# apple/ml-gmpi

Hardware: NVIDIA H100
Metric: MPI frames/s (96 planes, 1024^2) (higher is better)
Workload: dtype f32

## Files before the change

__graft_entry__.py:

```python
import os
import sys

ROOT = os.path.dirname(os.path.abspath(__file__))
for p in (ROOT, os.path.join(ROOT, "oracle")):
    if p not in sys.path:
        sys.path.insert(0, p)


def build() -> None:
    import ml_gmpi_b200
    from ml_gmpi_b200 import _build, _lib
    path = _build.build_library(force=False)
    assert os.path.exists(path)
    lib = _lib.load()
    assert lib.gmpi_abi_version() == _lib.ABI_VERSION
    import mpi_oracle
    mpi_oracle.build()
    print(f"built {path} and {mpi_oracle._SO}")


def smoke() -> None:
    import numpy as np
    import torch
    import ml_gmpi_b200 as g
    from ml_gmpi_b200 import synth
    import mpi_oracle

    assert torch.cuda.is_available(), "smoke() needs a CUDA device"
    dev = torch.device("cuda:0")
    from ml_gmpi_b200 import _lib
    N, T, IMG = 16, 256, 256
    case = synth.make_case(n_planes=N, tex=T, img=IMG, n_mpi=2, views_per_mpi=2, seed=7, device="cpu", last_alpha_one=True)
    case = case.to(dev)
    assert _lib.load().gmpi_mpi_render_fwd_plan(4, N, T, T, IMG, IMG, None, None) == _lib.PLAN_STAGED
    rgba = case.rgba.clone().requires_grad_(True)
    mpi = g.MPI(align_corners=True, validate="full")
# ... 23 lines not shown
```

ml_gmpi_b200/__init__.py:

```python
from . import _lib
from ._build import build_library
from .mpi import (MPI, MPIOutOfPlaneError, Occupancy, build_occupancy, check_range, expand_factored, render_frames,
                  render_views, render_views_factored, unorm8_to_float)

__all__ = ["MPI", "MPIOutOfPlaneError", "render_views", "render_views_factored", "render_frames", "expand_factored", "check_range",
           "build_library", "build_occupancy", "Occupancy", "unorm8_to_float"]
```

ml_gmpi_b200/_build.py:

```python
import os
import shutil
import subprocess

PKG_DIR = os.path.dirname(os.path.abspath(__file__))
CSRC = os.path.join(PKG_DIR, "csrc")
LIB_PATH = os.path.join(PKG_DIR, "libgmpi_mpi_render.so")
SOURCES = ["mpi_render.cu", "mpi_skip.cu", "mpi_u8.cu"]
HEADERS = ["mpi_common.cuh", "mpi_fwd_staged.cuh", "mpi_fwd_direct.cuh", "mpi_kernel_keys.cuh", "mpi_bwd_box.cuh", "mpi_bwd_direct.cuh",
           "mpi_range_check.cuh", "mpi_light.cuh", "mpi_debug.cuh", "tma_utils.cuh", os.path.join("..", "..", "include", "gmpi_mpi_render.h")]
NVCC_FLAGS = ["-gencode", "arch=compute_90a,code=sm_90a", "-lineinfo", "-O3", "-std=c++17", "-diag-suppress", "1886", "-shared",
              "-Xcompiler", "-fPIC"]


def nvcc_path():
    p = shutil.which("nvcc") or "/usr/local/cuda/bin/nvcc"
    if not os.path.exists(p):
        raise RuntimeError("nvcc not found; cannot build the sm_90a library")
    return p


def is_stale(path: str = LIB_PATH) -> bool:
    if not os.path.exists(path):
        return True
    t = os.path.getmtime(path)
    deps = [os.path.join(CSRC, s) for s in SOURCES + HEADERS] + [os.path.join(CSRC, f) for f in os.listdir(CSRC)]
    return any(os.path.getmtime(d) > t for d in deps if os.path.isfile(d))


def _nvcc(args, verbose):
    res = subprocess.run([nvcc_path()] + args + (["-Xptxas", "-v"] if verbose else []), cwd=CSRC, capture_output=True, text=True)
    if res.returncode != 0:
        raise RuntimeError("nvcc failed:\n" + res.stdout + res.stderr)
    if verbose:
        print(res.stdout + res.stderr)


def build_library(force: bool = False, verbose: bool = False) -> str:
    if force or is_stale(LIB_PATH):
        _nvcc(NVCC_FLAGS + ["-o", LIB_PATH] + SOURCES, verbose)
    return LIB_PATH
```

ml_gmpi_b200/csrc/mpi_fwd_staged.cuh:

```cuda
#pragma once
#include "mpi_common.cuh"
#include "tma_utils.cuh"
#include "mpi_kernel_keys.cuh"

namespace gmpi {

constexpr int kConsWarps = 15;
constexpr int kPairs = 2;
constexpr int kPix = 2 * kPairs;
constexpr int kTileW = 64, kTileH = kPairs * kConsWarps;
constexpr int kConsThreads = kConsWarps * 32, kStagedThreads = kConsThreads + 32;
constexpr int kStages = 3, kStreamStages = 2;
constexpr int kRowsPerOp = 4;
constexpr int kMaxBW = 88;
constexpr int kMaxBH = (((kTileH * 5) / 4 + 6 + kRowsPerOp - 1) / kRowsPerOp) * kRowsPerOp;
constexpr int kMinBW = 56, kBWStep = 8;
constexpr int kNumMaps = (kMaxBW - kMinBW) / kBWStep + 1;
constexpr int kMaxPlanesStaged = 512;
constexpr int kWideBW = 96;

__host__ __device__ constexpr int class_width(int k, bool wide = false) { return wide && k == kNumMaps - 1 ? kWideBW : kMinBW + k * kBWStep; }

template <class E, class B, CUtensorMapDataType kType>
struct ElemBase {
// ... 11 lines not shown
    static __device__ __forceinline__ bool out_of_unit(uint32_t b) { return b > 0x3f800000u && b != 0x80000000u; }
};
template <> struct ElemTraits<__half> : ElemBase<__half, uint16_t, CU_TENSOR_MAP_DATA_TYPE_FLOAT16> {
    static __host__ __device__ constexpr int staged_width(int bw, bool factored) { return bw + (factored ? 32 : 8); }
    static __device__ __forceinline__ bool nonfinite(uint32_t b) { return (b & 0x7c00u) == 0x7c00u; }
    static __device__ __forceinline__ bool out_of_unit(uint32_t b) { return b > 0x3c00u && b != 0x8000u; }
};
template <> struct ElemTraits<uint8_t> : ElemBase<uint8_t, uint8_t, CU_TENSOR_MAP_DATA_TYPE_UINT8> {
    static __host__ __device__ constexpr int staged_width(int bw, bool) { return (bw + 12 + 15) & ~15; }
};

struct TmaMaps {
    CUtensorMap m[kNumMaps];
    CUtensorMap m8[kNumMaps], m16[kNumMaps], m32[kNumMaps];
    CUtensorMap rgb[kNumMaps], bg[kNumMaps], a[kNumMaps];
    CUtensorMap t;
};

struct __align__(16) StageMeta {
    int cx, cy;
    int rows2;
    int sel;
};

typedef float2 f2;
__device__ __forceinline__ f2 splat(float a) { return make_float2(a, a); }
__device__ __forceinline__ f2 mul2(f2 a, f2 b) { return make_float2(__fmul_rn(a.x, b.x), __fmul_rn(a.y, b.y)); }
__device__ __forceinline__ f2 add2(f2 a, f2 b) { return make_float2(__fadd_rn(a.x, b.x), __fadd_rn(a.y, b.y)); }
__device__ __forceinline__ f2 fma2(f2 a, f2 b, f2 c) { return make_float2(__fmaf_rn(a.x, b.x, c.x), __fmaf_rn(a.y, b.y, c.y)); }
__device__ __forceinline__ f2 add2_rm(f2 a, f2 b) { return make_float2(__fadd_rd(a.x, b.x), __fadd_rd(a.y, b.y)); }
constexpr float kFloorMagic = 12582912.0f;
constexpr int kFloorMagicBits = 0x4b400000;
constexpr int kSelSlow = 0;

__device__ __forceinline__ f2 div2_by_rcp(f2 a, f2 nb, f2 y) {
    const f2 q0 = mul2(a, y);
    const f2 r = fma2(q0, nb, a);
    return fma2(r, y, q0);
}

struct RayPairs {
    f2 rx2[kPairs], ry2[kPairs];
    f2 nrz[kPairs], yrz[kPairs];
};
__device__ __forceinline__ void pack_ray_pairs(const RayConst (&rc)[kPix], RayPairs& rp) {
#pragma unroll
// ... 177 lines not shown
    }
    __host__ __device__ __forceinline__ void split(int t, int per_view, int& v, int& pos) const {
        if (group == 1) { v = t / per_view; pos = t - v * per_view; return; }
        const int per_group = per_view * group, g = t / per_group, rem = t - g * per_group;
        pos = rem / group;
        v = g * group + (rem - pos * group);
    }
    __host__ __device__ __forceinline__ bool at(int j, TileXY& r) const {
        int pos;
        if (j < n1) {
            split(cta + j * grid, full_per_view, r.v, pos);
            r.px0 = (pos % tiles_x) * kTileW; r.py0 = (pos / tiles_x) * tile_h;
            return true;
        }
        if (p_step == 0) return false;
        const int u = p_start + (j - n1) * p_step;
        if (u >= n_part) return false;
        split(u, tiles_x, r.v, pos);
        r.px0 = pos * kTileW; r.py0 = full_rows * tile_h;
        return true;
    }
};

__device__ __forceinline__ void consumer_idle_tile(uint64_t* s_full, uint64_t* s_empty, int N, int n_stages, int lane, int& c_stage,
                                                   uint32_t& c_phase) {
    for (int i = 0; i < N; ++i) {
        const int s = c_stage;
        const uint32_t ph = c_phase;
        if (++c_stage == n_stages) { c_stage = 0; c_phase ^= 1u; }
        mbar_wait(&s_full[s], ph);
        __syncwarp();
        mbar_arrive_if(&s_empty[s], lane == 0);
    }
}

template <bool kFactored, class E>
struct FwdRing {
    static constexpr int kTileRows = kTileH, kRingStages = kStages, kBoxMaxH = kMaxBH;
    static constexpr int kPlaneFloats = ElemTraits<E>::staged_width(kFactored ? kWideBW : kMaxBW, kFactored) * kMaxBH * 4;
    static constexpr int kStride = kPlaneFloats;
    static constexpr size_t kStageBytes = (size_t)kPlaneFloats * sizeof(E);
    static constexpr bool kReverse = false;
    static constexpr bool kSleepPolls = false;
    static constexpr bool kWideFact = kFactored;
    static constexpr bool kBinaryCopies = true;
    static constexpr int kColourCopyRows = kMaxBH / 2;
    static_assert(kStages * kStageBytes + (size_t)kMaxPlanesStaged * 32 + 1024 <= 227 * 1024, "the ring must fit one SM");
};
static_assert(kMaxBH % 2 == 0 && kMaxBH / kRowsPerOp < 16, "half-height colour copies; binary digits of the chunk count");
static_assert(FwdRing<false, float>::kPlaneFloats == 15488 && FwdRing<true, float>::kPlaneFloats == 16896 &&
              FwdRing<false, __half>::kPlaneFloats == 16896 && FwdRing<true, __half>::kPlaneFloats == 22528 &&
              FwdRing<false, uint8_t>::kPlaneFloats == 19712, "the staged forward's ring stages");
static_assert(FwdRing<false, uint8_t>::kStageBytes % 128 == 0, "uint8 ring stages stay 128-byte aligned");

__host__ __device__ __forceinline__ int binary_copy_of_lane(int n_chunks, int lane, int& before) {
    const int bit = 3 - lane;
    before = (n_chunks >> (bit + 1)) << (bit + 1);
    return ((n_chunks >> bit) & 1) << bit;
}

constexpr int kStopSlots = 4;
constexpr uint32_t kAllConsumers = (1u << kConsWarps) - 1u;
static_assert(kStages <= kStopSlots, "stop-word slots must cover the producer's lead");
__device__ unsigned long long g_early_stop_skipped;

constexpr int kOccB = 8;
constexpr int kSelEmpty = 1 << 24;
struct OccMap {
    const uint32_t* bits;
    int words, rows;
    unsigned long long* skipped;
};
__host__ __device__ __forceinline__ int occ_words(int Wt) { return ((Wt + kOccB - 1) / kOccB + 31) / 32; }
__host__ __device__ __forceinline__ int occ_rows(int Ht) { return (Ht + kOccB - 1) / kOccB; }

constexpr int kOccThreads = 32 * kOccB;

__device__ __forceinline__ void store_occ_word(bool occupied, uint32_t* dst, uint32_t* s_w) {
    const int warp = threadIdx.x >> 5, lane = threadIdx.x & 31;
    const uint32_t b = __ballot_sync(0xffffffffu, occupied);
    const uint32_t nib = ((b & 0xffu) ? 1u : 0u) | ((b & 0xff00u) ? 2u : 0u) | ((b & 0xff0000u) ? 4u : 0u) | ((b & 0xff000000u) ? 8u : 0u);
    if (lane == 0) s_w[warp] = nib << (4 * warp);
    __syncthreads();
    if (threadIdx.x == 0) {
        uint32_t w = 0;
#pragma unroll
        for (int k = 0; k < kOccThreads / 32; ++k) w |= s_w[k];
// ... 19 lines not shown
#endif
        acc |= word & (0xffffffffu >> (31 - hi)) & (0xffffffffu << lo);
    }
    return acc;
}

__device__ __forceinline__ bool box_vote(int cx, int cy, int bw2, int rows2, const CoordPairs& c) {
    const f2 magic = splat(kFloorMagic);
    bool inbox = true;
#pragma unroll
    for (int P = 0; P < kPairs; ++P) {
        const f2 tx = add2_rm(c.ix[P], magic), ty = add2_rm(c.iy[P], magic);
        inbox = inbox && (unsigned)(__float_as_int(tx.x) - cx) <= (unsigned)bw2 && (unsigned)(__float_as_int(tx.y) - cx) <= (unsigned)bw2 &&
                (unsigned)(__float_as_int(ty.x) - cy) <= (unsigned)rows2 && (unsigned)(__float_as_int(ty.y) - cy) <= (unsigned)rows2;
    }
    return __all_sync(0xffffffffu, inbox);
}

__device__ __forceinline__ uint32_t idle_consumer_warps(int py0, int H) {
    const int live = (H - py0 + kPairs - 1) / kPairs;
    return live >= kConsWarps ? 0u : kAllConsumers & ~((1u << live) - 1u);
}

template <bool kAlignCorners, class Ring, bool kFact, bool kES = false, class E = float, bool kSkip = false>
__device__ __forceinline__ void staged_producer(const RenderParams& p, const TmaMaps& maps, E* s_buf, StageMeta* s_meta,
                                            uint64_t* s_full, uint64_t* s_empty, const TileWalk* s_walk, int lane,
                                            int n_stages = Ring::kRingStages, uint32_t* s_stop = nullptr, OccMap occ = OccMap{}) {
    constexpr bool kReverse = Ring::kReverse;
    constexpr int kStride = Ring::kStride;
    constexpr int kTileH = Ring::kTileRows, kMaxBH = Ring::kBoxMaxH, kStageFloats = Ring::kPlaneFloats;
    constexpr uint32_t kTBytes = kReverse ? (uint32_t)(kTileW * kTileH * 4) : 0u;
    const int Ht = p.Ht, Wt = p.Wt, N = p.N;
    const float fWt = (float)Wt, fHt = (float)Ht;
    const float hsx = 0.5f * (float)(Wt - 1), hsy = 0.5f * (float)(Ht - 1);
    const size_t img = (size_t)p.H * p.W;
    if (lane < kNumMaps) {
        if (kFact) { tma_prefetch_desc(&maps.rgb[lane]); tma_prefetch_desc(&maps.a[lane]); }
        else { tma_prefetch_desc(&maps.m[lane]); tma_prefetch_desc(&maps.m8[lane]); tma_prefetch_desc(&maps.m16[lane]); tma_prefetch_desc(&maps.m32[lane]); }
    }
    int p_stage = 0;
    uint32_t p_phase = 0;
    uint32_t n_skipped = 0;
    uint32_t n_empty = 0;
    TileXY txy;
    for (int j = 0; s_walk->at(j, txy); ++j) {
        const int v = txy.v, px0 = txy.px0, py0 = txy.py0;
        const int m = __ldg(p.view2mpi + v);
        uint32_t* const stop_word = kES ? s_stop + (j & (kStopSlots - 1)) : nullptr;
        float ev[3], zd[3];
        load_eye_z(p, v, ev, zd);
        const int cx = min(px0 + ((lane & 1) ? kTileW - 1 : 0), p.W - 1);
        const int cy = min(py0 + ((lane & 2) ? kTileH - 1 : 0), p.H - 1);
        float crx, cry, crz;
        load_ray(p, v, cx, cy, img, crx, cry, crz);
        const RayConst rc = make_ray_const(crx, cry, crz, ev, zd);
        for (int ii = 0; ii < N; ++ii) {
            const int i = kReverse ? N - 1 - ii : ii;
            const int s = p_stage;
            const uint32_t ph = p_phase;
            if (++p_stage == n_stages) { p_stage = 0; p_phase ^= 1u; }
            const PlaneConst pc = make_plane_const(p.dhw + ((size_t)m * N + i) * 3, ev[2]);
            const TexCoord tc = plane_coord<kAlignCorners>(pc, rc, hsx, hsy, fWt, fHt);
            const bool finite = fabsf(tc.ix) < 1e9f && fabsf(tc.iy) < 1e9f;
            const bool all_finite = __all_sync(0xffffffffu, finite);
            const int fx = finite ? (int)floorf(tc.ix) : 0, fy = finite ? (int)floorf(tc.iy) : 0;
            const int xmin = __reduce_min_sync(0xffffffffu, fx), xmax = __reduce_max_sync(0xffffffffu, fx);
            const int ymin = __reduce_min_sync(0xffffffffu, fy), ymax = __reduce_max_sync(0xffffffffu, fy);
            const int bx0 = ((xmin - 1) >> 2) << 2, by0 = ymin - 1;
            const int need_w = xmax - bx0 + 3, need_h = ymax - ymin + 4;
            int mode = 0;
            constexpr bool kWide = kFact && Ring::kWideFact;
            if (!all_finite || need_w > kMaxBW || ((need_h + kRowsPerOp - 1) / kRowsPerOp) * kRowsPerOp > kMaxBH) mode = 2;
            else if (bx0 > Wt - 1 || bx0 + need_w - 1 < 0 || by0 > Ht - 1 || by0 + need_h - 1 < 0) mode = 1;
            const int k = mode != 0 ? 0 : kWide ? (need_w <= 64 ? 1 : 4) : max(0, (need_w - kMinBW + kBWStep - 1) / kBWStep);
            const int bw = class_width(k, kWide);
            const int bxs = ElemTraits<E>::staged_origin(bx0), sw = ElemTraits<E>::staged_width(bw, kWide);
            const int n_ops = mode == 0 ? (need_h + kRowsPerOp - 1) / kRowsPerOp : 0;
            const int rows = n_ops * kRowsPerOp;
            const bool testable = kSkip && mode == 0 && pc.fast != 0.0f;
            uint32_t occ_bits = 0u;
            if (testable) occ_bits = occ_box_bits(occ.bits + ((size_t)m * N + i) * occ.rows * occ.words, Ht, Wt, occ.words, bx0, by0, bw, rows, lane);
            if (Ring::kSleepPolls) mbar_wait_sleep(&s_empty[s], ph ^ 1);
            else mbar_wait(&s_empty[s], ph ^ 1);
            bool empty = false;
            if constexpr (kSkip) {
                empty = testable && !__any_sync(0xffffffffu, occ_bits != 0u);
                n_empty += empty ? 1u : 0u;
            }
            bool skip = false;
            if constexpr (kES) {
                if (ii == 0) {
                    if (lane == 0) *stop_word = idle_consumer_warps(py0, p.H);
                } else {
                    skip = __shfl_sync(0xffffffffu, *(volatile uint32_t*)stop_word, 0) == kAllConsumers;
                    n_skipped += skip ? 1u : 0u;
                }
            }
            const int n_copy = skip || empty ? 0 : n_ops;
            if (lane == 0) {
                StageMeta mt;
                mt.cx = kFloorMagicBits + bx0; mt.cy = kFloorMagicBits + by0;
                mt.rows2 = rows - 2;
                mt.sel = bw | (mode << 8) | ((mode == 0 && pc.fast != 0.0f ? (1 << k) : kSelSlow) << 16) | ((bx0 - bxs) << 10);
                if (kSkip && empty) mt.sel |= kSelEmpty;
                if constexpr (kReverse) {
                    const int ext_x = min(px0 + kTileW - 1, p.W - 1) - px0, ext_y = min(py0 + kTileH - 1, p.H - 1) - py0;
                    if (Ring::kMagLimit * (xmax - xmin - 1) < ext_x || Ring::kMagLimit * (ymax - ymin - 1) < ext_y) mt.sel &= 0xffff;
                }
                s_meta[s] = mt;
                const uint32_t tx = (uint32_t)((kFact ? kMaxBH : rows) * sw * (int)(4 * sizeof(E)));
                if (n_copy > 0 || kTBytes) mbar_arrive_expect_tx(&s_full[s], (n_copy > 0 ? tx : 0u) + kTBytes);
                else mbar_arrive(&s_full[s]);
                if (kReverse)
// ... 45 lines not shown
}

__device__ __forceinline__ void store_tile_pixels(const RenderParams& p, int v, size_t img, int pxb, int py, int lane, float (&o)[4]) {
    if (p.options & kOptVec4Stores) {
        quad_transpose(o, lane);
        const int k = lane & 3, px = pxb + 4 * (lane >> 2);
        if (px >= p.W || py >= p.H) return;
        const float4 val = make_float4(o[0], o[1], o[2], o[3]);
        const size_t pix = (size_t)py * p.W + px;
        if (p.n_peers > 0) {
            const size_t fo = ((size_t)(p.frame_offset + v) * 4 + k) * img + pix;
            for (int r = 0; r < p.n_peers; ++r) *reinterpret_cast<float4*>(p.peer_frames[r] + fo) = val;
        } else {
            float* dst = k < 3 ? p.color + ((size_t)v * 3 + k) * img + pix : p.depth + (size_t)v * img + pix;
            *reinterpret_cast<float4*>(dst) = val;
        }
        return;
    }
    const int px = pxb + lane;
    if (px >= p.W || py >= p.H) return;
    store_pixel(p, v, img, (size_t)py * p.W + px, o[0], o[1], o[2], o[3]);
}

template <bool kAlignCorners, bool kEmitT, bool kFactored, bool kES, class E = float, bool kSkip = false>
__device__ __forceinline__ void fwd_staged_body(const RenderParams& p, const TmaMaps& maps, const int tiles_x, const int ring_stages,
                                                uint32_t* s_stop, OccMap occ = OccMap{}) {
    extern __shared__ __align__(1024) unsigned char smem_raw[];
    E* s_buf = reinterpret_cast<E*>(smem_raw);
    using Ring = FwdRing<kFactored, E>;
    static_assert(!(kFactored && std::is_same<E, uint8_t>::value), "uint8 MPIs are expanded");
    constexpr int kStages = Ring::kRingStages;
    const int n_stages = kFactored ? kStages : ring_stages;
    constexpr int kRingFloats = Ring::kPlaneFloats;
    constexpr int kAOff = kFactored ? 3 * (kRingFloats / 4) : 0;
    PlaneConst* s_pc = reinterpret_cast<PlaneConst*>(smem_raw + (size_t)n_stages * kRingFloats * sizeof(E));
    __shared__ StageMeta s_meta[kStages];
    __shared__ __align__(8) uint64_t s_full[kStages], s_empty[kStages];
    __shared__ TileWalk s_walk;

    const int warp = threadIdx.x >> 5, lane = threadIdx.x & 31;
    if (threadIdx.x == 0) {
        s_walk.init(tiles_x, p.H, p.V, (int)blockIdx.x, (int)gridDim.x, kTileH, p.view_group);
        for (int s = 0; s < n_stages; ++s) {
            mbar_init(&s_full[s], 1);
            mbar_init(&s_empty[s], kConsWarps);
        }
        fence_mbar_init();
    }
    __syncthreads();

    const int Ht = p.Ht, Wt = p.Wt, N = p.N;
    const float fWt = (float)Wt, fHt = (float)Ht;
    float hsx = 0.5f * (float)(Wt - 1), hsy = 0.5f * (float)(Ht - 1);
    asm volatile("" : "+f"(hsx), "+f"(hsy));
    int lane_ = lane;
    asm volatile("" : "+r"(lane_));
    const size_t img = (size_t)p.H * p.W;

    if (warp == kConsWarps) {
        staged_producer<kAlignCorners, Ring, kFactored, kES, E, kSkip>(p, maps, s_buf, s_meta, s_full, s_empty, &s_walk, lane, n_stages,
                                                                        s_stop, occ);
    } else {
        const bool check_last = (p.options & GMPI_CHECK_LAST_PLANE) != 0;
        const bool minus1_1 = (p.options & GMPI_COLOR_MINUS1_1) != 0;
        const float tau = kES ? p.early_stop : 0.0f;
        int c_stage = 0;
        uint32_t c_phase = 0;
        uint32_t flag = 0;
        const size_t tex = (size_t)Ht * Wt;
        int v_table = -1;
        TileXY txy;
        for (int j = 0; s_walk.at(j, txy); ++j) {
            const int v = txy.v, px0 = txy.px0, py0 = txy.py0;
            const int m = __ldg(p.view2mpi + v);
            float ev[3], zd[3];
            load_eye_z(p, v, ev, zd);
            if (v != v_table) {
                consumer_bar_sync<kConsThreads>();
                const float eye0_z = __ldg(p.eye0 + 2);
                for (int i = threadIdx.x; i < N; i += kConsThreads) {
                    const float* dp = p.dhw + ((size_t)m * N + i) * 3;
                    s_pc[i] = make_plane_const(dp, ev[2]);
                    if (!(__ldg(dp) >= eye0_z)) flag |= GMPI_FLAG_PLANE_BEHIND_EYE;
                }
                consumer_bar_sync<kConsThreads>();
                v_table = v;
            }
            if (py0 + kPairs * warp >= p.H) {
                consumer_idle_tile(s_full, s_empty, N, n_stages, lane, c_stage, c_phase);
                continue;
            }
            RayConst rc[kPix];
            RayPairs rp;
            bool rays_fast = (in_safe_range(ev[0]) || ev[0] == 0.0f) && (in_safe_range(ev[1]) || ev[1] == 0.0f);
#pragma unroll
            for (int q = 0; q < kPix; ++q) {
                const int px = min(px0 + lane + 32 * (q & 1), p.W - 1), py = min(py0 + kPairs * warp + (q >> 1), p.H - 1);
                float qx, qy, qz;
                load_ray(p, v, px, py, img, qx, qy, qz);
                rc[q] = make_ray_const(qx, qy, qz, ev, zd);
                rays_fast = rays_fast && rc[q].fast && fabsf(rc[q].rx2) <= 0x1p40f && fabsf(rc[q].ry2) <= 0x1p40f;
            }
            pack_ray_pairs(rc, rp);
            const f2 ex2 = splat(rc[0].ex2), ey2 = splat(rc[0].ey2), hsx2 = splat(hsx), hsy2 = splat(hsy);
            const bool warp_fast = __all_sync(0xffffffffu, rays_fast);
            f2 T[kPairs], cr[kPairs], cg[kPairs], cb[kPairs], cws[kPairs];
#pragma unroll
            for (int P = 0; P < kPairs; ++P) { T[P] = splat(1.f); cr[P] = cg[P] = cb[P] = cws[P] = splat(0.f); }
            PlaneConst pc_next = s_pc[0];
            bool warp_stopped = false;
            uint32_t* const stop_word = kES ? s_stop + (j & (kStopSlots - 1)) : nullptr;
            for (int i = 0; i < N; ++i) {
                const int s = c_stage;
                const uint32_t ph = c_phase;
                if (++c_stage == n_stages) { c_stage = 0; c_phase ^= 1u; }
                const PlaneConst pcc = pc_next;
                pc_next = s_pc[min(i + 1, N - 1)];
                CoordPairs cc;
                if (warp_fast && !warp_stopped) coords_pairs<kAlignCorners>(pcc, rp, ex2, ey2, hsx2, hsy2, fWt, fHt, cc);
                if (kEmitT) {
                    float* ts = p.transmittance + ((size_t)v * N + i) * img;
#pragma unroll
                    for (int q = 0; q < kPix; ++q) {
                        const int px = px0 + lane + 32 * (q & 1), py = py0 + kPairs * warp + (q >> 1);
                        if (px < p.W && py < p.H) ts[(size_t)py * p.W + px] = (q & 1) ? T[q >> 1].y : T[q >> 1].x;
                    }
                }
                mbar_wait(&s_full[s], ph);
                const StageMeta mt = s_meta[s];
                const E* sb = s_buf + s * kRingFloats + ((mt.sel >> 10) & ElemTraits<E>::kOriginMask);
                const int sel = mt.sel;
                bool done = warp_stopped;
                if (warp_fast && !done) {
                    if (kSkip && (sel & kSelEmpty)) {
// ... 37 lines not shown
                            const float w00 = wx0 * wy0, w01 = wx1 * wy0, w10 = wx0 * wy1, w11 = wx1 * wy1;
                            const E* t0 = sb + ((int)ryy * bw4 + (int)rxx);
                            const E* t1 = t0 + bw4;
                            r = fmaf(to_f32(t1[1]), w11, fmaf(to_f32(t1[0]), w10, fmaf(to_f32(t0[1]), w01, to_f32(t0[0]) * w00)));
                            g = fmaf(to_f32(t1[bws + 1]), w11, fmaf(to_f32(t1[bws]), w10, fmaf(to_f32(t0[bws + 1]), w01, to_f32(t0[bws]) * w00)));
                            b = fmaf(to_f32(t1[2 * bws + 1]), w11,
                                     fmaf(to_f32(t1[2 * bws]), w10, fmaf(to_f32(t0[2 * bws + 1]), w01, to_f32(t0[2 * bws]) * w00)));
                            a = fmaf(to_f32(t1[3 * bws + 1]), w11,
                                     fmaf(to_f32(t1[3 * bws]), w10, fmaf(to_f32(t0[3 * bws + 1]), w01, to_f32(t0[3 * bws]) * w00)));
                        } else if (coord_hits(tc.ix, tc.iy, fWt, fHt)) {
                            const float4 sv = sample_plane_any<kFactored, E>(p, plane, m, i, tex, tc.ix, tc.iy);
                            r = sv.x; g = sv.y; b = sv.z; a = sv.w;
                        } else {
                            continue;
                        }
                        const float w = a * Ts[q];
                        crs[q] = fmaf(w, r, crs[q]);
                        cgs[q] = fmaf(w, g, cgs[q]);
                        cbs[q] = fmaf(w, b, cbs[q]);
                        cwss[q] = fmaf(w, tc.scale, cwss[q]);
                        Ts[q] -= w;
                    }
                }
                if constexpr (kES) {
                    if (!warp_stopped) {
                        bool st = true;
#pragma unroll
                        for (int P = 0; P < kPairs; ++P) st = st && fabsf(T[P].x) <= tau && fabsf(T[P].y) <= tau;
                        warp_stopped = __all_sync(0xffffffffu, st);
                        if (warp_stopped && i + 1 < N && lane_ == 0) atomicOr(stop_word, 1u << warp);
                    }
                }
                __syncwarp();
                mbar_arrive_if(&s_empty[s], lane_ == 0);
            }
            if (check_last) {
                const PlaneConst pcl = s_pc[N - 1];
#pragma unroll
                for (int q = 0; q < kPix; ++q) {
                    RayConst rg = rc[q];
                    rg.fast = false;
                    const TexCoord tc = plane_coord<kAlignCorners>(pcl, rg, hsx, hsy, fWt, fHt);
                    if (!(tc.u >= -1.0f && tc.u <= 1.0f && tc.v >= -1.0f && tc.v <= 1.0f)) flag |= GMPI_FLAG_LAST_PLANE_OOB;
                }
            }
#pragma unroll
            for (int q = 0; q < kPix; ++q) {
                float o[4];
                o[0] = (q & 1) ? cr[q >> 1].y : cr[q >> 1].x; o[1] = (q & 1) ? cg[q >> 1].y : cg[q >> 1].x;
                o[2] = (q & 1) ? cb[q >> 1].y : cb[q >> 1].x;
                o[3] = ((q & 1) ? cws[q >> 1].y : cws[q >> 1].x) * rc[q].dz;
                if (minus1_1) {
                    o[0] = fmaf(2.0f, o[0], -1.0f); o[1] = fmaf(2.0f, o[1], -1.0f); o[2] = fmaf(2.0f, o[2], -1.0f);
                }
                store_tile_pixels(p, v, img, px0 + 32 * (q & 1), py0 + kPairs * warp + (q >> 1), lane, o);
            }
        }
        if (flag) atomicOr(p.flags, flag);
    }
}

template <uint32_t K>
__global__ void __launch_bounds__(kStagedThreads, 1)
mpi_fwd_staged_kernel(const RenderParams p, const __grid_constant__ TmaMaps maps, const int tiles_x, const int tiles_y,
                      const int ring_stages) {
    using T = KeyTraits<K>;
    static_assert((K & (kKeyStaged | kKeyBwd | kKeySkip)) == kKeyStaged, "a staged forward key without skipping");
    if constexpr (T::kES) {
        __shared__ uint32_t s_stop[kStopSlots];
        fwd_staged_body<T::kAlignCorners, T::kEmitT, T::kFactored, true, typename T::Elem>(p, maps, tiles_x, ring_stages, s_stop);
    } else {
        fwd_staged_body<T::kAlignCorners, T::kEmitT, T::kFactored, false, typename T::Elem>(p, maps, tiles_x, ring_stages, nullptr);
    }
}

template <uint32_t K>
__global__ void __launch_bounds__(kStagedThreads, 1)
mpi_fwd_skip_kernel(const RenderParams p, const __grid_constant__ TmaMaps maps, const int tiles_x, const int tiles_y,
                    const int ring_stages, const OccMap occ) {
    using T = KeyTraits<K>;
    static_assert((K & (kKeyStaged | kKeyBwd | kKeySkip | kKeyEmit)) == (kKeyStaged | kKeySkip), "a skipping forward key");
    if constexpr (T::kES) {
        __shared__ uint32_t s_stop[kStopSlots];
        fwd_staged_body<T::kAlignCorners, false, T::kFactored, true, typename T::Elem, true>(p, maps, tiles_x, ring_stages, s_stop, occ);
    } else {
        fwd_staged_body<T::kAlignCorners, false, T::kFactored, false, typename T::Elem, true>(p, maps, tiles_x, ring_stages, nullptr, occ);
    }
}

}
```

ml_gmpi_b200/csrc/mpi_kernel_keys.cuh:

```cuda
#pragma once
#include <cuda_runtime.h>
#include <cuda_fp16.h>
#include <stdint.h>
#include <type_traits>

namespace gmpi {

enum : uint32_t {
    kKeyAC = 1, kKeyFac = 2, kKeyEmit = 4, kKeyES = 8, kKeyF16 = 16, kKeyStaged = 32, kKeyBwd = 64, kKeyDet = 128, kKeySkip = 256,
    kKeyU8 = 512
};

template <uint32_t K>
struct KeyTraits {
    static constexpr bool kAlignCorners = (K & kKeyAC) != 0, kFactored = (K & kKeyFac) != 0, kEmitT = (K & kKeyEmit) != 0,
                          kES = (K & kKeyES) != 0, kSkip = (K & kKeySkip) != 0, kDet = (K & kKeyDet) != 0;
    using Elem = std::conditional_t<(K & kKeyU8) != 0, uint8_t, std::conditional_t<(K & kKeyF16) != 0, __half, float>>;
};

struct RenderKernel {
    uint32_t key;
    const void* kernel;
    template <class... A>
    RenderKernel(uint32_t k, void (*f)(A...)) : key(k), kernel(reinterpret_cast<const void*>(f)) {}
};

struct KernelUnit {
    const RenderKernel *begin, *end;
    cudaError_t (*stage_counters)(unsigned long long** early_stop, unsigned long long** empty);
};
extern const KernelUnit render_unit;
extern const KernelUnit skip_unit;
extern const KernelUnit u8_unit;

}

extern "C" {
__global__ void gmpi_occ_expanded_f32(const uint32_t*, uint32_t*, uint32_t*, int, int, int, int, int);
__global__ void gmpi_occ_expanded_f16(const uint16_t*, uint32_t*, uint32_t*, int, int, int, int, int);
// ... 6 lines not shown
```

ml_gmpi_b200/csrc/mpi_render.cu:

```cuda
#include <cuda_runtime.h>
#include <stdarg.h>
#include <stdint.h>
#include <math.h>
#include <stdio.h>
#include <string.h>

#include <algorithm>
#include <atomic>
#include <iterator>
#include <mutex>
#include <tuple>
#include <type_traits>
#include <utility>

#include "../../include/gmpi_mpi_render.h"
#include "mpi_common.cuh"
#include "mpi_fwd_staged.cuh"
#include "mpi_bwd_box.cuh"
#include "mpi_light.cuh"
#include "mpi_fwd_direct.cuh"
#include "mpi_bwd_direct.cuh"
#include "mpi_range_check.cuh"
#include "mpi_debug.cuh"
#include "mpi_kernel_keys.cuh"

namespace gmpi {

static thread_local char g_err[512] = "";

static int fail(int code, const char* fmt, ...) {
    va_list ap;
    va_start(ap, fmt);
    vsnprintf(g_err, sizeof(g_err), fmt, ap);
// ... 206 lines not shown
    {kKeyF16 | kKeyES, mpi_fwd_direct_kernel<kKeyF16 | kKeyES>},
    {kKeyF16 | kKeyES | kKeyAC, mpi_fwd_direct_kernel<kKeyF16 | kKeyES | kKeyAC>},
    {kKeyBwd | kKeyDet | kKeyAC, mpi_bwd_direct_det_kernel<kKeyBwd | kKeyDet | kKeyAC>},
    {kKeyBwd | kKeyDet, mpi_bwd_direct_det_kernel<kKeyBwd | kKeyDet>},
    {kKeyBwd | kKeyAC, mpi_bwd_direct_kernel<kKeyBwd | kKeyAC>},
    {kKeyBwd, mpi_bwd_direct_kernel<kKeyBwd>},
    {kKeyBwd | kKeyDet | kKeyStaged | kKeyAC | kKeyFac, mpi_bwd_box_det_kernel<kKeyBwd | kKeyDet | kKeyStaged | kKeyAC | kKeyFac>},
    {kKeyBwd | kKeyDet | kKeyStaged | kKeyFac, mpi_bwd_box_det_kernel<kKeyBwd | kKeyDet | kKeyStaged | kKeyFac>},
    {kKeyBwd | kKeyDet | kKeyStaged | kKeyAC, mpi_bwd_box_det_kernel<kKeyBwd | kKeyDet | kKeyStaged | kKeyAC>},
    {kKeyBwd | kKeyDet | kKeyStaged, mpi_bwd_box_det_kernel<kKeyBwd | kKeyDet | kKeyStaged>},
    {kKeyBwd | kKeyStaged | kKeyAC | kKeyFac, mpi_bwd_box_kernel<kKeyBwd | kKeyStaged | kKeyAC | kKeyFac>},
    {kKeyBwd | kKeyStaged | kKeyFac, mpi_bwd_box_kernel<kKeyBwd | kKeyStaged | kKeyFac>},
    {kKeyBwd | kKeyStaged | kKeyAC, mpi_bwd_box_kernel<kKeyBwd | kKeyStaged | kKeyAC>},
    {kKeyBwd | kKeyStaged, mpi_bwd_box_kernel<kKeyBwd | kKeyStaged>},
};

static cudaError_t render_stage_counters(unsigned long long** early_stop, unsigned long long** empty) {
    *empty = nullptr;
    return cudaGetSymbolAddress(reinterpret_cast<void**>(early_stop), g_early_stop_skipped);
}

const KernelUnit gmpi::render_unit = {std::begin(kRenderKernels), std::end(kRenderKernels), render_stage_counters};

static const KernelUnit& key_unit(uint32_t key) {
    return (key & kKeyU8) ? u8_unit : (key & kKeySkip) ? skip_unit : render_unit;
}

static const void* render_kernel(uint32_t key) {
    const KernelUnit& u = key_unit(key);
    const RenderKernel* k = std::find_if(u.begin, u.end, [key](const RenderKernel& r) { return r.key == key; });
    return k == u.end ? nullptr : k->kernel;
}

struct Launch {
    uint32_t key = 0;
    dim3 grid, block;
    size_t smem = 0;
    long tiles = 0;
    RenderParams p;
    TmaMaps maps;
    int ints[3] = {};
    OccMap om;
    DetAcc da;
    void* args[6] = {&p};
    int n_args = 1;
    explicit Launch(const RenderParams& q) : p(q) {
        if (!p.eye0) p.eye0 = p.cam ? p.cam + 13 : p.eye;
        if (p.view_group < 1) p.view_group = 1;
    }
    Launch(const Launch&) = delete;
    void arg(void* a) { args[n_args++] = a; }
};

static int launch_args(const void* kernel, dim3 grid, dim3 block, size_t smem, cudaStream_t st, void** args) {
    if (smem > 48 * 1024) GMPI_CUDA_OK(cudaFuncSetAttribute(kernel, cudaFuncAttributeMaxDynamicSharedMemorySize, (int)smem));
    cudaLaunchConfig_t cfg = {grid, block, smem, st, nullptr, 0};
    GMPI_CUDA_OK(cudaLaunchKernelExC(&cfg, kernel, args));
    return GMPI_OK;
}

template <class... P, class... A>
static int launch_kernel(void (*kernel)(P...), dim3 grid, dim3 block, size_t smem, cudaStream_t st, A&&... a) {
    static_assert(sizeof...(P) == sizeof...(A), "one argument per kernel parameter");
    std::tuple<P...> params(std::forward<A>(a)...);
    return std::apply([&](P&... x) {
        void* arg_addrs[] = {&x...};
        return launch_args(reinterpret_cast<const void*>(kernel), grid, block, smem, st, arg_addrs);
    }, params);
}

static int launch(Launch& l, cudaStream_t st) { return launch_args(render_kernel(l.key), l.grid, l.block, l.smem, st, l.args); }

static int persistent_grid(Launch& l, int tile_h) {
    const RenderParams& p = l.p;
    int sms = 0;
    if (int rc = device_attr(cudaDevAttrMultiProcessorCount, &sms)) return rc;
    l.ints[0] = (p.W + kTileW - 1) / kTileW;
    l.ints[1] = (p.H + tile_h - 1) / tile_h;
    l.tiles = (long)l.ints[0] * l.ints[1] * p.V;
    l.grid = dim3((unsigned)(l.tiles < sms ? l.tiles : sms));
    l.arg(&l.maps);
    l.arg(&l.ints[0]);
    l.arg(&l.ints[1]);
    return GMPI_OK;
}

static size_t fwd_staged_smem(const RenderParams& p, int stages) {
    const size_t ring = with_mpi_elem(p.options, [&](auto e) {
        using E = typename decltype(e)::Elem;
        return factored(p) ? kStages * FwdRing<true, E>::kStageBytes : stages * FwdRing<false, E>::kStageBytes;
    });
    return ring + (size_t)kMaxPlanesStaged * 32;
}

// ... 24 lines not shown
    GMPI_CUDA_OK(cudaDeviceSynchronize());
    *skipped = 0;
    if (counter) GMPI_CUDA_OK(cudaMemcpy(skipped, counter, sizeof(unsigned long long), cudaMemcpyDeviceToHost));
    *walked = g_stages_walked[s].load(std::memory_order_relaxed);
    return GMPI_OK;
}

static int fwd_launch(Launch& l, const uint32_t* occ) {
    const RenderParams& p = l.p;
    const bool fac = factored(p);
    uint32_t key = ((p.options & GMPI_ALIGN_CORNERS) ? kKeyAC : 0) | ((p.options & GMPI_EARLY_STOP) ? kKeyES : 0) |
                   ((p.options & GMPI_MPI_F16) ? kKeyF16 : 0) | ((p.options & GMPI_MPI_U8) ? kKeyU8 : 0);
    int rc = GMPI_OK;
    if (fwd_why(p) == 0) {
        if (encode_mpi_maps(l.maps, p, kMaxBH, FwdRing<true, float>::kColourCopyRows, fac) == 0) {
            int l2 = 0;
            if ((rc = persistent_grid(l, kTileH)) != 0) return rc;
            if ((rc = device_attr(cudaDevAttrL2CacheSize, &l2)) != 0) return rc;
            const int forced_stages = g_fwd_stages.load(std::memory_order_relaxed);
            l.ints[2] = forced_stages ? forced_stages : fwd_ring_stages(p, l2);
            l.block = dim3(kStagedThreads);
            l.smem = fwd_staged_smem(p, l.ints[2]);
            l.arg(&l.ints[2]);
            key |= kKeyStaged | (fac ? kKeyFac : 0) | (occ ? kKeySkip : 0) | (p.transmittance ? kKeyEmit : 0);
            l.key = key;
            if (!occ) return GMPI_OK;
            l.om = OccMap{occ, occ_words(p.Wt), occ_rows(p.Ht), nullptr};
            l.arg(&l.om);
            return stage_counter(kSkipStats, key_unit(key), &l.om.skipped);
        }
        if (g_fwd_variant.load(std::memory_order_relaxed) == 2) return fail(GMPI_ERR_CUDA, "cuTensorMapEncodeTiled failed");
    }
    l.p.options &= ~kOptVec4Stores;
    l.smem = sizeof(PlaneConst) * (size_t)p.N;
    if (l.smem > 200 * 1024) return fail(GMPI_ERR_UNSUPPORTED, "N=%d planes exceed the shared-memory plane table", p.N);
    l.block = dim3(kFwdTileW, kFwdTileH);
    l.grid = dim3((p.W + kFwdTileW - 1) / kFwdTileW, (p.H + kFwdTileH - 1) / kFwdTileH, p.V);
    if (l.grid.y > 65535) return fail(GMPI_ERR_UNSUPPORTED, "image height %d too large", p.H);
    if (p.V > 65535) return fail(GMPI_ERR_UNSUPPORTED, "V=%d views exceed one launch of the direct kernel (65535); split the batch", p.V);
    l.key = key;
    return GMPI_OK;
}

static int launch_fwd(RenderParams p, cudaStream_t st, const uint32_t* occ = nullptr) {
    if (p.V == 0) return GMPI_OK;
    if (p.W % 4 == 0 && !p.video_rgb && (p.n_peers > 0 || (aligned16(p.color) && aligned16(p.depth)))) p.options |= kOptVec4Stores;
    Launch l(p);
// ... 708 lines not shown
```

Measured before the change: 1660.

## Stop forward compositing once transmittance is provably below float resolution

Adds an 'absorb' variant of the staged forward kernel, used whenever transmittance is not emitted. Consumer warps test whether the remaining transmittance, scaled by a bound on depth and colour, can no longer change the accumulated colour or depth in float precision. When every warp in a tile stops, the producer stops issuing TMA loads for the remaining planes and posts an end marker, so no further plane data is fetched or composited. The variants are compiled into a separate cubin loaded at runtime through the CUDA library API, which adds module-loading and mangled-name lookup failure modes and more per-plane checks.

```diff
diff --git a/__graft_entry__.py b/__graft_entry__.py
--- a/__graft_entry__.py
+++ b/__graft_entry__.py
@@ -11,7 +11,8 @@
     import ml_gmpi_b200
     from ml_gmpi_b200 import _build, _lib
     path = _build.build_library(force=False)
-    assert os.path.exists(path)
+    module = _build.build_fwd_module(force=False)
+    assert os.path.exists(path) and os.path.exists(module)
     lib = _lib.load()
     assert lib.gmpi_abi_version() == _lib.ABI_VERSION
     import mpi_oracle
diff --git a/ml_gmpi_b200/__init__.py b/ml_gmpi_b200/__init__.py
--- a/ml_gmpi_b200/__init__.py
+++ b/ml_gmpi_b200/__init__.py
@@ -1,7 +1,14 @@
 from . import _lib
-from ._build import build_library
+from . import _build
 from .mpi import (MPI, MPIOutOfPlaneError, Occupancy, build_occupancy, check_range, expand_factored, render_frames,
                   render_views, render_views_factored, unorm8_to_float)
 
+
+
+def build_library(force: bool = False, verbose: bool = False) -> str:
+    _build.build_fwd_module(force, verbose)
+    return _build.build_library(force, verbose)
+
+
 __all__ = ["MPI", "MPIOutOfPlaneError", "render_views", "render_views_factored", "render_frames", "expand_factored", "check_range",
            "build_library", "build_occupancy", "Occupancy", "unorm8_to_float"]
diff --git a/ml_gmpi_b200/_build.py b/ml_gmpi_b200/_build.py
--- a/ml_gmpi_b200/_build.py
+++ b/ml_gmpi_b200/_build.py
@@ -6,6 +6,8 @@
 CSRC = os.path.join(PKG_DIR, "csrc")
 LIB_PATH = os.path.join(PKG_DIR, "libgmpi_mpi_render.so")
 SOURCES = ["mpi_render.cu", "mpi_skip.cu", "mpi_u8.cu"]
+MODULE_SOURCE = "mpi_fwd_absorb.cu"
+MODULE_PATH = os.path.join(PKG_DIR, "gmpi_fwd_absorb.cubin")
 HEADERS = ["mpi_common.cuh", "mpi_fwd_staged.cuh", "mpi_fwd_direct.cuh", "mpi_kernel_keys.cuh", "mpi_bwd_box.cuh", "mpi_bwd_direct.cuh",
            "mpi_range_check.cuh", "mpi_light.cuh", "mpi_debug.cuh", "tma_utils.cuh", os.path.join("..", "..", "include", "gmpi_mpi_render.h")]
 NVCC_FLAGS = ["-gencode", "arch=compute_90a,code=sm_90a", "-lineinfo", "-O3", "-std=c++17", "-diag-suppress", "1886", "-shared",
@@ -39,3 +41,10 @@
     if force or is_stale(LIB_PATH):
         _nvcc(NVCC_FLAGS + ["-o", LIB_PATH] + SOURCES, verbose)
     return LIB_PATH
+
+
+def build_fwd_module(force: bool = False, verbose: bool = False) -> str:
+    if force or is_stale(MODULE_PATH):
+        flags = [f for f in NVCC_FLAGS if f not in ("-shared", "-Xcompiler", "-fPIC")]
+        _nvcc(flags + ["-cubin", "-o", MODULE_PATH, MODULE_SOURCE], verbose)
+    return MODULE_PATH
diff --git a/ml_gmpi_b200/csrc/mpi_fwd_absorb.cu b/ml_gmpi_b200/csrc/mpi_fwd_absorb.cu
--- /dev/null
+++ b/ml_gmpi_b200/csrc/mpi_fwd_absorb.cu
@@ -0,0 +1,24 @@
+#include "../../include/gmpi_mpi_render.h"
+#include "mpi_common.cuh"
+#include "mpi_fwd_staged.cuh"
+
+namespace gmpi {
+
+#define GMPI_STAGED(K) template __global__ void mpi_fwd_staged_kernel<(K) | kKeyAbsorb>(const RenderParams, const __grid_constant__ TmaMaps, \
+                                                                                        const int, const int, const int);
+#define GMPI_SKIP(K) template __global__ void mpi_fwd_skip_kernel<(K) | kKeyAbsorb>(const RenderParams, const __grid_constant__ TmaMaps, \
+                                                                                    const int, const int, const int, const OccMap);
+#define GMPI_AC_ES(M, B) M(B) M((B) | kKeyAC) M((B) | kKeyES) M((B) | kKeyAC | kKeyES)
+
+GMPI_AC_ES(GMPI_STAGED, kKeyStaged)
+GMPI_AC_ES(GMPI_STAGED, kKeyStaged | kKeyFac)
+GMPI_AC_ES(GMPI_STAGED, kKeyStaged | kKeyF16)
+GMPI_AC_ES(GMPI_STAGED, kKeyStaged | kKeyF16 | kKeyFac)
+GMPI_AC_ES(GMPI_STAGED, kKeyStaged | kKeyU8)
+GMPI_AC_ES(GMPI_SKIP, kKeyStaged | kKeySkip)
+GMPI_AC_ES(GMPI_SKIP, kKeyStaged | kKeySkip | kKeyFac)
+GMPI_AC_ES(GMPI_SKIP, kKeyStaged | kKeySkip | kKeyF16)
+GMPI_AC_ES(GMPI_SKIP, kKeyStaged | kKeySkip | kKeyF16 | kKeyFac)
+GMPI_AC_ES(GMPI_SKIP, kKeyStaged | kKeySkip | kKeyU8)
+
+}
diff --git a/ml_gmpi_b200/csrc/mpi_fwd_staged.cuh b/ml_gmpi_b200/csrc/mpi_fwd_staged.cuh
--- a/ml_gmpi_b200/csrc/mpi_fwd_staged.cuh
+++ b/ml_gmpi_b200/csrc/mpi_fwd_staged.cuh
@@ -57,6 +57,7 @@
     int rows2;
     int sel;
 };
+constexpr int kSelEnd = 1 << 25;
 
 typedef float2 f2;
 __device__ __forceinline__ f2 splat(float a) { return make_float2(a, a); }
@@ -280,15 +281,18 @@
     }
 };
 
-__device__ __forceinline__ void consumer_idle_tile(uint64_t* s_full, uint64_t* s_empty, int N, int n_stages, int lane, int& c_stage,
-                                                   uint32_t& c_phase) {
+template <bool kEnd = false>
+__device__ __forceinline__ void consumer_idle_tile(uint64_t* s_full, uint64_t* s_empty, const StageMeta* s_meta, int N, int n_stages,
+                                                   int lane, int& c_stage, uint32_t& c_phase) {
     for (int i = 0; i < N; ++i) {
         const int s = c_stage;
         const uint32_t ph = c_phase;
         if (++c_stage == n_stages) { c_stage = 0; c_phase ^= 1u; }
         mbar_wait(&s_full[s], ph);
+        const bool end = kEnd && (s_meta[s].sel & kSelEnd) != 0;
         __syncwarp();
         mbar_arrive_if(&s_empty[s], lane == 0);
+        if (end) break;
     }
 }
 
@@ -319,8 +323,27 @@
 
 constexpr int kStopSlots = 4;
 constexpr uint32_t kAllConsumers = (1u << kConsWarps) - 1u;
-static_assert(kStages <= kStopSlots, "stop-word slots must cover the producer's lead");
+static_assert(1 + (kStages - 2) / 2 < kStopSlots, "stop-word slots must cover the producer's lead");
 __device__ unsigned long long g_early_stop_skipped;
+
+constexpr float kAbsorbK = 4.0f;
+constexpr float kAbsorbPre = 0x1p-27f;
+__device__ __forceinline__ float half_spacing_below(float x) {
+    return __int_as_float((__float_as_int(x) & 0x7f800000) - (25 << 23));
+}
+template <bool kES>
+__device__ __forceinline__ bool pixel_stopped(float T, float r, float g, float b, float ws, float S, float tau) {
+    if (kES && fabsf(T) <= tau) return true;
+    const float kt = kAbsorbK * fabsf(T);
+    return kt < half_spacing_below(fminf(fabsf(r), fminf(fabsf(g), fabsf(b)))) && kt * S < half_spacing_below(ws);
+}
+__device__ __forceinline__ float scale_bound(const PlaneConst* s_pc, int N, const RayConst (&rc)[kPix], int lane) {
+    uint32_t z = 0u, y = 0u;
+    for (int i = lane; i < N; i += 32) z = max(z, __float_as_uint(fabsf(s_pc[i].z_diff)));
+#pragma unroll
+    for (int q = 0; q < kPix; ++q) y = max(y, __float_as_uint(fabsf(rc[q].yrz)));
+    return __uint_as_float(__reduce_max_sync(0xffffffffu, z)) * __uint_as_float(__reduce_max_sync(0xffffffffu, y));
+}
 
 constexpr int kOccB = 8;
 constexpr int kSelEmpty = 1 << 24;
@@ -386,7 +409,7 @@
     return live >= kConsWarps ? 0u : kAllConsumers & ~((1u << live) - 1u);
 }
 
-template <bool kAlignCorners, class Ring, bool kFact, bool kES = false, class E = float, bool kSkip = false>
+template <bool kAlignCorners, class Ring, bool kFact, bool kES = false, class E = float, bool kSkip = false, bool kEnd = false>
 __device__ __forceinline__ void staged_producer(const RenderParams& p, const TmaMaps& maps, E* s_buf, StageMeta* s_meta,
                                             uint64_t* s_full, uint64_t* s_empty, const TileWalk* s_walk, int lane,
                                             int n_stages = Ring::kRingStages, uint32_t* s_stop = nullptr, OccMap occ = OccMap{}) {
@@ -406,11 +429,12 @@
     uint32_t p_phase = 0;
     uint32_t n_skipped = 0;
     uint32_t n_empty = 0;
+    uint32_t recent = 0;
     TileXY txy;
     for (int j = 0; s_walk->at(j, txy); ++j) {
         const int v = txy.v, px0 = txy.px0, py0 = txy.py0;
         const int m = __ldg(p.view2mpi + v);
-        uint32_t* const stop_word = kES ? s_stop + (j & (kStopSlots - 1)) : nullptr;
+        uint32_t* const stop_word = kES || kEnd ? s_stop + (j & (kStopSlots - 1)) : nullptr;
         float ev[3], zd[3];
         load_eye_z(p, v, ev, zd);
         const int cx = min(px0 + ((lane & 1) ? kTileW - 1 : 0), p.W - 1);
@@ -446,13 +470,35 @@
             if (testable) occ_bits = occ_box_bits(occ.bits + ((size_t)m * N + i) * occ.rows * occ.words, Ht, Wt, occ.words, bx0, by0, bw, rows, lane);
             if (Ring::kSleepPolls) mbar_wait_sleep(&s_empty[s], ph ^ 1);
             else mbar_wait(&s_empty[s], ph ^ 1);
+            if constexpr (kEnd) {
+                if (ii == 0) {
+                    if (lane == 0) {
+                        stop_word[0] = idle_consumer_warps(py0, p.H);
+                        stop_word[kStopSlots] = 0u;
+                    }
+                } else if (__shfl_sync(0xffffffffu, *(volatile uint32_t*)stop_word, 0) == kAllConsumers) {
+                    if constexpr (kSkip) {
+                        __threadfence_block();
+                        const int last = (int)__shfl_sync(0xffffffffu, *(volatile uint32_t*)(stop_word + kStopSlots), 0);
+                        n_empty -= __popc(recent & ((1u << (ii - 1 - last)) - 1u));
+                    }
+                    if (lane == 0) {
+                        s_meta[s].sel = kSelEnd;
+                        mbar_arrive(&s_full[s]);
+                    }
+                    __syncwarp();
+                    n_skipped += N - ii;
+                    break;
+                }
+            }
             bool empty = false;
             if constexpr (kSkip) {
                 empty = testable && !__any_sync(0xffffffffu, occ_bits != 0u);
                 n_empty += empty ? 1u : 0u;
+                if constexpr (kEnd) recent = (recent << 1) | (empty ? 1u : 0u);
             }
             bool skip = false;
-            if constexpr (kES) {
+            if constexpr (kES && !kEnd) {
                 if (ii == 0) {
                     if (lane == 0) *stop_word = idle_consumer_warps(py0, p.H);
                 } else {
@@ -544,7 +590,7 @@
     store_pixel(p, v, img, (size_t)py * p.W + px, o[0], o[1], o[2], o[3]);
 }
 
-template <bool kAlignCorners, bool kEmitT, bool kFactored, bool kES, class E = float, bool kSkip = false>
+template <bool kAlignCorners, bool kEmitT, bool kFactored, bool kES, class E = float, bool kSkip = false, bool kAbsorb = false>
 __device__ __forceinline__ void fwd_staged_body(const RenderParams& p, const TmaMaps& maps, const int tiles_x, const int ring_stages,
                                                 uint32_t* s_stop, OccMap occ = OccMap{}) {
     extern __shared__ __align__(1024) unsigned char smem_raw[];
@@ -578,10 +624,11 @@
     int lane_ = lane;
     asm volatile("" : "+r"(lane_));
     const size_t img = (size_t)p.H * p.W;
+    constexpr bool kStop = kAbsorb && !kEmitT;
 
     if (warp == kConsWarps) {
-        staged_producer<kAlignCorners, Ring, kFactored, kES, E, kSkip>(p, maps, s_buf, s_meta, s_full, s_empty, &s_walk, lane, n_stages,
-                                                                        s_stop, occ);
+        staged_producer<kAlignCorners, Ring, kFactored, kES, E, kSkip, kStop>(p, maps, s_buf, s_meta, s_full, s_empty, &s_walk, lane,
+                                                                               n_stages, s_stop, occ);
     } else {
         const bool check_last = (p.options & GMPI_CHECK_LAST_PLANE) != 0;
         const bool minus1_1 = (p.options & GMPI_COLOR_MINUS1_1) != 0;
@@ -609,7 +656,7 @@
                 v_table = v;
             }
             if (py0 + kPairs * warp >= p.H) {
-                consumer_idle_tile(s_full, s_empty, N, n_stages, lane, c_stage, c_phase);
+                consumer_idle_tile<kStop>(s_full, s_empty, s_meta, N, n_stages, lane, c_stage, c_phase);
                 continue;
             }
             RayConst rc[kPix];
@@ -631,7 +678,8 @@
             for (int P = 0; P < kPairs; ++P) { T[P] = splat(1.f); cr[P] = cg[P] = cb[P] = cws[P] = splat(0.f); }
             PlaneConst pc_next = s_pc[0];
             bool warp_stopped = false;
-            uint32_t* const stop_word = kES ? s_stop + (j & (kStopSlots - 1)) : nullptr;
+            uint32_t* const stop_word = kES || kStop ? s_stop + (j & (kStopSlots - 1)) : nullptr;
+            const float depth_bound = kStop ? scale_bound(s_pc, N, rc, lane) : 0.0f;
             for (int i = 0; i < N; ++i) {
                 const int s = c_stage;
                 const uint32_t ph = c_phase;
@@ -715,7 +763,7 @@
                         Ts[q] -= w;
                     }
                 }
-                if constexpr (kES) {
+                if constexpr (kES && !kStop) {
                     if (!warp_stopped) {
                         bool st = true;
 #pragma unroll
@@ -724,8 +772,31 @@
                         if (warp_stopped && i + 1 < N && lane_ == 0) atomicOr(stop_word, 1u << warp);
                     }
                 }
+                if constexpr (kStop) {
+                    if (!warp_stopped) {
+                        float tm = fmaxf(fabsf(T[0].x), fabsf(T[0].y));
+#pragma unroll
+                        for (int P = 1; P < kPairs; ++P) tm = fmaxf(tm, fmaxf(fabsf(T[P].x), fabsf(T[P].y)));
+                        if (__all_sync(0xffffffffu, tm < kAbsorbPre || (kES && tm <= tau))) {
+                            bool st = true;
+#pragma unroll
+                            for (int P = 0; P < kPairs; ++P)
+                                st = st && pixel_stopped<kES>(T[P].x, cr[P].x, cg[P].x, cb[P].x, cws[P].x, depth_bound, tau) &&
+                                     pixel_stopped<kES>(T[P].y, cr[P].y, cg[P].y, cb[P].y, cws[P].y, depth_bound, tau);
+                            warp_stopped = __all_sync(0xffffffffu, st);
+                            if (warp_stopped && i + n_stages < N && lane_ == 0) {
+                                if (kSkip) {
+                                    atomicMax(stop_word + kStopSlots, (uint32_t)i);
+                                    __threadfence_block();
+                                }
+                                atomicOr(stop_word, 1u << warp);
+                            }
+                        }
+                    }
+                }
                 __syncwarp();
                 mbar_arrive_if(&s_empty[s], lane_ == 0);
+                if (kStop && (sel & kSelEnd)) break;
             }
             if (check_last) {
                 const PlaneConst pcl = s_pc[N - 1];
@@ -759,7 +830,11 @@
                       const int ring_stages) {
     using T = KeyTraits<K>;
     static_assert((K & (kKeyStaged | kKeyBwd | kKeySkip)) == kKeyStaged, "a staged forward key without skipping");
-    if constexpr (T::kES) {
+    static_assert(!(T::kAbsorb && T::kEmitT), "the training forward walks every plane");
+    if constexpr (T::kAbsorb) {
+        __shared__ uint32_t s_stop[2 * kStopSlots];
+        fwd_staged_body<T::kAlignCorners, false, T::kFactored, T::kES, typename T::Elem, false, true>(p, maps, tiles_x, ring_stages, s_stop);
+    } else if constexpr (T::kES) {
         __shared__ uint32_t s_stop[kStopSlots];
         fwd_staged_body<T::kAlignCorners, T::kEmitT, T::kFactored, true, typename T::Elem>(p, maps, tiles_x, ring_stages, s_stop);
     } else {
@@ -773,7 +848,10 @@
                     const int ring_stages, const OccMap occ) {
     using T = KeyTraits<K>;
     static_assert((K & (kKeyStaged | kKeyBwd | kKeySkip | kKeyEmit)) == (kKeyStaged | kKeySkip), "a skipping forward key");
-    if constexpr (T::kES) {
+    if constexpr (T::kAbsorb) {
+        __shared__ uint32_t s_stop[2 * kStopSlots];
+        fwd_staged_body<T::kAlignCorners, false, T::kFactored, T::kES, typename T::Elem, true, true>(p, maps, tiles_x, ring_stages, s_stop, occ);
+    } else if constexpr (T::kES) {
         __shared__ uint32_t s_stop[kStopSlots];
         fwd_staged_body<T::kAlignCorners, false, T::kFactored, true, typename T::Elem, true>(p, maps, tiles_x, ring_stages, s_stop, occ);
     } else {
diff --git a/ml_gmpi_b200/csrc/mpi_kernel_keys.cuh b/ml_gmpi_b200/csrc/mpi_kernel_keys.cuh
--- a/ml_gmpi_b200/csrc/mpi_kernel_keys.cuh
+++ b/ml_gmpi_b200/csrc/mpi_kernel_keys.cuh
@@ -8,13 +8,14 @@
 
 enum : uint32_t {
     kKeyAC = 1, kKeyFac = 2, kKeyEmit = 4, kKeyES = 8, kKeyF16 = 16, kKeyStaged = 32, kKeyBwd = 64, kKeyDet = 128, kKeySkip = 256,
-    kKeyU8 = 512
+    kKeyU8 = 512, kKeyAbsorb = 1024
 };
 
 template <uint32_t K>
 struct KeyTraits {
     static constexpr bool kAlignCorners = (K & kKeyAC) != 0, kFactored = (K & kKeyFac) != 0, kEmitT = (K & kKeyEmit) != 0,
-                          kES = (K & kKeyES) != 0, kSkip = (K & kKeySkip) != 0, kDet = (K & kKeyDet) != 0;
+                          kES = (K & kKeyES) != 0, kSkip = (K & kKeySkip) != 0, kDet = (K & kKeyDet) != 0,
+                          kAbsorb = (K & kKeyAbsorb) != 0;
     using Elem = std::conditional_t<(K & kKeyU8) != 0, uint8_t, std::conditional_t<(K & kKeyF16) != 0, __half, float>>;
 };
 
diff --git a/ml_gmpi_b200/csrc/mpi_render.cu b/ml_gmpi_b200/csrc/mpi_render.cu
--- a/ml_gmpi_b200/csrc/mpi_render.cu
+++ b/ml_gmpi_b200/csrc/mpi_render.cu
@@ -1,4 +1,5 @@
 #include <cuda_runtime.h>
+#include <dlfcn.h>
 #include <stdarg.h>
 #include <stdint.h>
 #include <math.h>
@@ -9,6 +10,7 @@
 #include <atomic>
 #include <iterator>
 #include <mutex>
+#include <string>
 #include <tuple>
 #include <type_traits>
 #include <utility>
@@ -261,11 +263,67 @@
 
 const KernelUnit gmpi::render_unit = {std::begin(kRenderKernels), std::end(kRenderKernels), render_stage_counters};
 
+static std::mutex g_absorb_mu;
+static cudaLibrary_t g_absorb_lib = nullptr;
+static cudaKernel_t g_absorb_kernels[2 * kKeyAbsorb];
+static std::string g_absorb_path;
+
+static cudaError_t absorb_module(cudaLibrary_t* lib) {
+    if (!g_absorb_lib) {
+        Dl_info info;
+        if (!dladdr(reinterpret_cast<void*>(&absorb_module), &info) || !info.dli_fname) return cudaErrorFileNotFound;
+        const std::string so = info.dli_fname;
+        g_absorb_path = so.substr(0, so.find_last_of('/') + 1) + "gmpi_fwd_absorb.cubin";
+        const cudaError_t e = cudaLibraryLoadFromFile(&g_absorb_lib, g_absorb_path.c_str(), nullptr, nullptr, 0, nullptr, nullptr, 0);
+        if (e != cudaSuccess) { g_absorb_lib = nullptr; return e; }
+    }
+    *lib = g_absorb_lib;
+    return cudaSuccess;
+}
+
+static const void* absorb_kernel(uint32_t key) {
+    std::lock_guard<std::mutex> guard(g_absorb_mu);
+    if (key >= 2 * kKeyAbsorb) return nullptr;
+    if (!g_absorb_kernels[key]) {
+        cudaLibrary_t lib;
+        cudaError_t e = absorb_module(&lib);
+        if (e != cudaSuccess) {
+            fail(GMPI_ERR_CUDA, "cannot load the forward kernel module %s: %s", g_absorb_path.c_str(), cudaGetErrorString(e));
+            return nullptr;
+        }
+        char name[128];
+        snprintf(name, sizeof name, (key & kKeySkip) ? "_ZN4gmpi19mpi_fwd_skip_kernelILj%uEEEvNS_12RenderParamsENS_7TmaMapsEiiiNS_6OccMapE"
+                                                     : "_ZN4gmpi21mpi_fwd_staged_kernelILj%uEEEvNS_12RenderParamsENS_7TmaMapsEiii", key);
+        if ((e = cudaLibraryGetKernel(&g_absorb_kernels[key], lib, name)) != cudaSuccess) {
+            g_absorb_kernels[key] = nullptr;
+            fail(GMPI_ERR_CUDA, "kernel %s not in %s: %s", name, g_absorb_path.c_str(), cudaGetErrorString(e));
+            return nullptr;
+        }
+    }
+    return reinterpret_cast<const void*>(g_absorb_kernels[key]);
+}
+
+static cudaError_t absorb_counters(const KernelUnit& plain, unsigned long long** early_stop, unsigned long long** empty) {
+    unsigned long long* unused = nullptr;
+    cudaError_t e = plain.stage_counters(&unused, empty);
+    if (e != cudaSuccess) return e;
+    std::lock_guard<std::mutex> guard(g_absorb_mu);
+    cudaLibrary_t lib;
+    if ((e = absorb_module(&lib)) != cudaSuccess) return e;
+    size_t bytes = 0;
+    return cudaLibraryGetGlobal(reinterpret_cast<void**>(early_stop), &bytes, lib, "_ZN4gmpi20g_early_stop_skippedE");
+}
+static cudaError_t absorb_counters_f(unsigned long long** es, unsigned long long** empty) { return absorb_counters(skip_unit, es, empty); }
+static cudaError_t absorb_counters_u8(unsigned long long** es, unsigned long long** empty) { return absorb_counters(u8_unit, es, empty); }
+static const KernelUnit absorb_unit = {nullptr, nullptr, absorb_counters_f}, absorb_u8_unit = {nullptr, nullptr, absorb_counters_u8};
+
 static const KernelUnit& key_unit(uint32_t key) {
+    if (key & kKeyAbsorb) return (key & kKeyU8) ? absorb_u8_unit : absorb_unit;
     return (key & kKeyU8) ? u8_unit : (key & kKeySkip) ? skip_unit : render_unit;
 }
 
 static const void* render_kernel(uint32_t key) {
+    if (key & kKeyAbsorb) return absorb_kernel(key);
     const KernelUnit& u = key_unit(key);
     const RenderKernel* k = std::find_if(u.begin, u.end, [key](const RenderKernel& r) { return r.key == key; });
     return k == u.end ? nullptr : k->kernel;
@@ -308,7 +366,11 @@
     }, params);
 }
 
-static int launch(Launch& l, cudaStream_t st) { return launch_args(render_kernel(l.key), l.grid, l.block, l.smem, st, l.args); }
+static int launch(Launch& l, cudaStream_t st) {
+    const void* kernel = render_kernel(l.key);
+    if (!kernel && (l.key & kKeyAbsorb)) return GMPI_ERR_CUDA;
+    return launch_args(kernel, l.grid, l.block, l.smem, st, l.args);
+}
 
 static int persistent_grid(Launch& l, int tile_h) {
     const RenderParams& p = l.p;
@@ -379,7 +441,7 @@
             l.block = dim3(kStagedThreads);
             l.smem = fwd_staged_smem(p, l.ints[2]);
             l.arg(&l.ints[2]);
-            key |= kKeyStaged | (fac ? kKeyFac : 0) | (occ ? kKeySkip : 0) | (p.transmittance ? kKeyEmit : 0);
+            key |= kKeyStaged | (fac ? kKeyFac : 0) | (occ ? kKeySkip : 0) | (p.transmittance ? kKeyEmit : kKeyAbsorb);
             l.key = key;
             if (!occ) return GMPI_OK;
             l.om = OccMap{occ, occ_words(p.Wt), occ_rows(p.Ht), nullptr};
```

Result: faster. 2869 (median of 6 runs) (+72.8%).
